# bnosac/image

Measured on NVIDIA H100. Metric: Mpixels/sec (Harris+Canny+HOG) at 4K frames, higher is better.
Workload: dtype f32 (Harris, FHOG) / f64 (Canny, Harris certification)

## Files before the change

image_b200/csrc/canny.cu:

```cuda
#include "common.cuh"
#include <cmath>
#include <vector>

namespace b2f {

constexpr int CANNY_MAXR = 64;
struct CannyTaps {
  double w[CANNY_MAXR + 1];
  int R;
};

constexpr int CB_TW = 32, CB_TH = 64, CB_NT = 256;

__device__ __forceinline__ int wrap_index(int p, int n) {
  while (p < 0) p += n;
  while (p >= n) p -= n;
  return p;
}

template <int RT>
__global__ void __launch_bounds__(CB_NT, 3)
canny_blur_kernel(const unsigned char *__restrict__ frames, float *__restrict__ out, int nx, int ny,
                  const __grid_constant__ CannyTaps tx, const __grid_constant__ CannyTaps ty) {
  extern __shared__ __align__(16) double smem_d[];
// ... 21 lines not shown
        for (int q = 0; q < MAXC; q++) b[k][q] = (lane + 32 * q < TILE_W) ? __ldg(row + cofs[q]) : (unsigned char)0;
      }
#pragma unroll
      for (int k = 0; k < RBATCH; k++) {
        const int r = r0 + (CB_NT / 32) * k;
        if (r < TILE_H) {
#pragma unroll
          for (int q = 0; q < MAXC; q++) if (lane + 32 * q < TILE_W) tile[r * TP + lane + 32 * q] = (double)b[k][q];
        }
      }
    }
    for (int r = warp; r < TILE_H; r += CB_NT / 32) {
      const unsigned char *row = src + (size_t)wrap_index(y0 - RY + r, ny) * nx;
      for (int c = lane + 32 * MAXC; c < TILE_W; c += 32) tile[r * TP + c] = (double)__ldg(row + wrap_index(x0 - RX + c, nx));
    }
  }
  __syncthreads();
  if (RT) {
    constexpr int RR = RT ? RT : 1;
    constexpr int NV = 4 + 2 * RR;
    for (int it = threadIdx.x; it < TILE_H * (CB_TW / 4); it += CB_NT) {
      const int r = it / (CB_TW / 4), g = it - r * (CB_TW / 4);
      const double *p = tile + r * TP + 4 * g;
      double v[NV];
#pragma unroll
      for (int q = 0; q < NV / 2; q++) { double2 t = *reinterpret_cast<const double2 *>(p + 2 * q); v[2 * q] = t.x; v[2 * q + 1] = t.y; }
      double o[4];
#pragma unroll
      for (int j = 0; j < 4; j++) {
        double acc = __dmul_rn(tx.w[0], v[j + RR]);
#pragma unroll
        for (int k = 1; k <= RR; k++) acc = __fma_rn(tx.w[k], __dadd_rn(v[j + RR - k], v[j + RR + k]), acc);
        o[j] = acc;
      }
      double *d = rowbuf + r * CB_TW + 4 * g;
      *reinterpret_cast<double2 *>(d) = make_double2(o[0], o[1]);
      *reinterpret_cast<double2 *>(d + 2) = make_double2(o[2], o[3]);
    }
  } else {
    for (int r = warp; r < TILE_H; r += CB_NT / 32) {
      const double *p = tile + r * TP + lane + RX;
      double acc = __dmul_rn(tx.w[0], p[0]);
      for (int k = 1; k <= RX; k++) acc = __fma_rn(tx.w[k], __dadd_rn(p[-k], p[k]), acc);
      rowbuf[r * CB_TW + lane] = acc;
    }
  }
  __syncthreads();
  {
    const int c = lane;
    const int gx = x0 + c;
    float *dst = out + (size_t)blockIdx.z * nx * ny;
    if (RT) {
      constexpr int RB = 8;
      constexpr int RR = RT ? RT : 1;
      for (int rg = warp; rg < CB_TH / RB; rg += CB_NT / 32) {
        double v[RB + 2 * RR];
#pragma unroll
        for (int q = 0; q < RB + 2 * RR; q++) v[q] = rowbuf[(rg * RB + q) * CB_TW + c];
#pragma unroll
        for (int j = 0; j < RB; j++) {
          double acc = __dmul_rn(ty.w[0], v[j + RR]);
#pragma unroll
          for (int k = 1; k <= RR; k++) acc = __fma_rn(ty.w[k], __dadd_rn(v[j + RR - k], v[j + RR + k]), acc);
          int gy = y0 + rg * RB + j;
          if (gx < nx && gy < ny) dst[(size_t)gy * nx + gx] = __double2float_rn(acc);
        }
      }
    } else {
      for (int r = warp; r < CB_TH; r += CB_NT / 32) {
        const double *p = rowbuf + (r + RY) * CB_TW + c;
        double acc = __dmul_rn(ty.w[0], p[0]);
        for (int k = 1; k <= RY; k++) acc = __fma_rn(ty.w[k], __dadd_rn(p[-k * CB_TW], p[k * CB_TW]), acc);
        int gy = y0 + r;
        if (gx < nx && gy < ny) dst[(size_t)gy * nx + gx] = __double2float_rn(acc);
      }
    }
  }
}

__device__ __forceinline__ double u32_to_double(unsigned s) {
  return __dadd_rn(__hiloint2double(0x43300000, (int)s), -4503599627370496.0);
}

template <int RR>
__global__ void __launch_bounds__(256)
canny_blur_rows_kernel(const unsigned char *__restrict__ frames, double *__restrict__ rowsum, int nx, int ny,
                       const __grid_constant__ CannyTaps tx) {
  const int y = blockIdx.y;
  const int x4 = (blockIdx.x * blockDim.x + threadIdx.x) * 4;
  if (x4 >= nx) return;
  const unsigned char *row = frames + ((size_t)blockIdx.z * ny + y) * nx;
  constexpr int LEAD = (RR + 3) & ~3;
  constexpr int NW = (LEAD + 4 + RR + 3) / 4;
  unsigned char b[NW * 4];
  const bool fast = (nx & 3) == 0 && NW * 4 <= nx && (reinterpret_cast<uintptr_t>(frames) & 3) == 0;
  if (fast) {
    const unsigned *w = reinterpret_cast<const unsigned *>(row);
    const int nw = nx >> 2, w0 = (x4 - LEAD) >> 2;
    unsigned v[NW];
#pragma unroll
    for (int q = 0; q < NW; q++) {
      int wi = w0 + q;
      wi += wi < 0 ? nw : 0;
      wi -= wi >= nw ? nw : 0;
      v[q] = __ldg(w + wi);
    }
#pragma unroll
    for (int q = 0; q < NW; q++) { b[4 * q] = v[q] & 0xff; b[4 * q + 1] = (v[q] >> 8) & 0xff; b[4 * q + 2] = (v[q] >> 16) & 0xff; b[4 * q + 3] = v[q] >> 24; }
  } else {
#pragma unroll
    for (int q = 0; q < NW * 4; q++) b[q] = __ldg(row + wrap_index(x4 - LEAD + q, nx));
  }
  double o[4];
#pragma unroll
  for (int j = 0; j < 4; j++) {
    const int c = LEAD + j;
    double acc = __dmul_rn(tx.w[0], u32_to_double(b[c]));
#pragma unroll
    for (int k = 1; k <= RR; k++) acc = __fma_rn(tx.w[k], u32_to_double((unsigned)b[c - k] + (unsigned)b[c + k]), acc);
    o[j] = acc;
  }
  double *d = rowsum + ((size_t)blockIdx.z * ny + y) * nx + x4;
  if (x4 + 3 < nx && (nx & 1) == 0) {
    *reinterpret_cast<double2 *>(d) = make_double2(o[0], o[1]);
    *reinterpret_cast<double2 *>(d + 2) = make_double2(o[2], o[3]);
  } else {
#pragma unroll
    for (int j = 0; j < 4; j++) if (x4 + j < nx) d[j] = o[j];
  }
}

constexpr int CC_TW = 32, CC_TH = 128;
template <int RR>
__global__ void __launch_bounds__(256)
canny_blur_cols_kernel(const double *__restrict__ rowsum, float *__restrict__ out, int nx, int ny,
                       const __grid_constant__ CannyTaps ty) {
  extern __shared__ __align__(16) double smem_d[];
  constexpr int TILE_H = CC_TH + 2 * RR;
  const int x0 = blockIdx.x * CC_TW, y0 = blockIdx.y * CC_TH;
  const double *src = rowsum + (size_t)blockIdx.z * nx * ny;
  const int lane = threadIdx.x & 31, warp = threadIdx.x >> 5;
  const int gx = x0 + lane;
  const int cx = min(gx, nx - 1);
  {
    constexpr int RBATCH = 10;
    for (int r0 = warp; r0 < TILE_H; r0 += 8 * RBATCH) {
      double v[RBATCH];
#pragma unroll
      for (int k = 0; k < RBATCH; k++) {
        const int r = min(r0 + 8 * k, TILE_H - 1);
        v[k] = __ldg(src + (size_t)wrap_index(y0 - RR + r, ny) * nx + cx);
      }
#pragma unroll
      for (int k = 0; k < RBATCH; k++) { const int r = r0 + 8 * k; if (r < TILE_H) smem_d[r * CC_TW + lane] = v[k]; }
    }
  }
  __syncthreads();
  float *dst = out + (size_t)blockIdx.z * nx * ny;
  constexpr int RB = 8;
  for (int rg = warp; rg < CC_TH / RB; rg += 8) {
    double v[RB + 2 * RR];
#pragma unroll
    for (int q = 0; q < RB + 2 * RR; q++) v[q] = smem_d[(rg * RB + q) * CC_TW + lane];
#pragma unroll
    for (int j = 0; j < RB; j++) {
      double acc = __dmul_rn(ty.w[0], v[j + RR]);
#pragma unroll
      for (int k = 1; k <= RR; k++) acc = __fma_rn(ty.w[k], __dadd_rn(v[j + RR - k], v[j + RR + k]), acc);
      const int gy = y0 + rg * RB + j;
      if (gx < nx && gy < ny) dst[(size_t)gy * nx + gx] = __double2float_rn(acc);
    }
  }
}

struct TapList { const int *coord; const double *weight; int n; int sym; };
__global__ void canny_blur_generic_rows(const unsigned char *__restrict__ frames, double *__restrict__ tmp, int nx, int ny,
                                        TapList t) {
  int x = blockIdx.x * blockDim.x + threadIdx.x, y = blockIdx.y;
  if (x >= nx) return;
  const unsigned char *src = frames + (size_t)blockIdx.z * nx * ny + (size_t)y * nx;
  double acc;
  if (t.sym) {
    const int R = t.n / 2;
    acc = __dmul_rn(t.weight[R], (double)src[x]);
    for (int k = 1; k <= R; k++)
      acc = __fma_rn(t.weight[R + k], __dadd_rn((double)src[wrap_index(x - k, nx)], (double)src[wrap_index(x + k, nx)]), acc);
  } else {
    acc = 0;
    for (int i = 0; i < t.n; i++) acc = __fma_rn(t.weight[i], (double)src[wrap_index(x - t.coord[i], nx)], acc);
  }
  tmp[(size_t)blockIdx.z * nx * ny + (size_t)y * nx + x] = acc;
}
__global__ void canny_blur_generic_cols(const double *__restrict__ tmp, float *__restrict__ out, int nx, int ny, TapList t) {
  int x = blockIdx.x * blockDim.x + threadIdx.x, y = blockIdx.y;
  if (x >= nx) return;
  const double *src = tmp + (size_t)blockIdx.z * nx * ny + x;
  double acc;
  if (t.sym) {
    const int R = t.n / 2;
    acc = __dmul_rn(t.weight[R], src[(size_t)y * nx]);
    for (int k = 1; k <= R; k++)
      acc = __fma_rn(t.weight[R + k], __dadd_rn(src[(size_t)wrap_index(y - k, ny) * nx], src[(size_t)wrap_index(y + k, ny) * nx]), acc);
  } else {
    acc = 0;
    for (int i = 0; i < t.n; i++) acc = __fma_rn(t.weight[i], src[(size_t)wrap_index(y - t.coord[i], ny) * nx], acc);
  }
  out[(size_t)blockIdx.z * nx * ny + (size_t)y * nx + x] = __double2float_rn(acc);
}

__device__ __forceinline__ double hypot_glibc(double x, double y) {
  x = fabs(x); y = fabs(y);
  double ax = x < y ? y : x, ay = x < y ? x : y;
  if (ax >= __dmul_rn(ay, 0x1p54)) return __dadd_rn(ax, ay);
  double h = __dsqrt_rn(__dadd_rn(__dmul_rn(ax, ax), __dmul_rn(ay, ay)));
  double t1, t2;
  if (h <= __dmul_rn(2.0, ay)) {
    double delta = __dsub_rn(h, ay);
    t1 = __dmul_rn(ax, __dsub_rn(__dmul_rn(2.0, delta), ax));
    t2 = __dmul_rn(__dsub_rn(delta, __dmul_rn(2.0, __dsub_rn(ax, ay))), delta);
  } else {
    double delta = __dsub_rn(h, ax);
    t1 = __dmul_rn(__dmul_rn(2.0, delta), __dsub_rn(ax, __dmul_rn(2.0, ay)));
    t2 = __dadd_rn(__dmul_rn(__dsub_rn(__dmul_rn(4.0, delta), ay), ay), __dmul_rn(delta, delta));
  }
  return __dsub_rn(h, __ddiv_rn(__dadd_rn(t1, t2), __dmul_rn(2.0, h)));
}

constexpr int CG_T = 32, CG_NT = 256;

constexpr int SG_DW = CG_T + 4;
constexpr int SG_DH = CG_T + 5;
constexpr int SG_GW = CG_T + 2;
constexpr int SG_GH = CG_T + 3;
constexpr int SG_K = 5;
__device__ __forceinline__ float rcp_approx(float x) { float r; asm("rcp.approx.ftz.f32 %0, %1;" : "=f"(r) : "f"(x)); return r; }
__device__ __forceinline__ float sqrt_approx(float x) { float r; asm("sqrt.approx.ftz.f32 %0, %1;" : "=f"(r) : "f"(x)); return r; }

__device__ __forceinline__ void exact_hv2(const float *d, int accGrad, double &h, double &v) {
#define DD(dx, dy) ((double)d[(dy) * SG_DW + (dx)])
  if (accGrad) {
    h = __dmul_rn(2.0, __dsub_rn(DD(1, 0), DD(-1, 0)));
    h = __dadd_rn(h, DD(1, 1)); h = __dsub_rn(h, DD(-1, 1)); h = __dadd_rn(h, DD(1, -1)); h = __dsub_rn(h, DD(-1, -1));
    v = __dmul_rn(2.0, __dsub_rn(DD(0, 1), DD(0, -1)));
    v = __dadd_rn(v, DD(1, 1)); v = __dsub_rn(v, DD(1, -1)); v = __dadd_rn(v, DD(-1, 1)); v = __dsub_rn(v, DD(-1, -1));
  } else {
    h = __dsub_rn(DD(1, 0), DD(-1, 0));
    v = __dsub_rn(DD(0, 1), DD(0, -1));
  }
#undef DD
}

template <bool ACC>
__global__ void __launch_bounds__(CG_NT)
canny_grad_nms_spec2_kernel(const float *__restrict__ data, unsigned *__restrict__ emask, unsigned *__restrict__ smask, int nx, int ny,
                            int low_thr, int high_thr, unsigned long long *__restrict__ fallback_count) {
  __shared__ __align__(16) float sd[SG_DH * SG_DW];
  __shared__ float fg[SG_GH * SG_GW];
  __shared__ float2 fhv[SG_GH * SG_GW];
  __shared__ float s_emax[CG_NT / 32];
  __shared__ __align__(4) unsigned char scls[CG_T * CG_T];
  __shared__ unsigned short squeue[CG_T * CG_T];
  __shared__ double sg2[28 * 9];
  __shared__ int qn;
  const int x0 = blockIdx.x * CG_T, y0 = blockIdx.y * CG_T;
  const float *src = data + (size_t)blockIdx.z * nx * ny;
  const int lane = threadIdx.x & 31, warp = threadIdx.x >> 5;
  if (threadIdx.x == 0) qn = 0;
  if (x0 >= 2 && y0 >= 2 && x0 + SG_DW - 2 <= nx && y0 + SG_DH - 2 <= ny && (nx & 1) == 0) {
    const float *org = src + (size_t)(y0 - 2) * nx + (x0 - 2);
    float2 v[3];
    int so[3];
#pragma unroll
    for (int k = 0; k < 3; k++) {
      const int u = threadIdx.x + k * CG_NT;
      const int row = u / (SG_DW / 2), cu = u - row * (SG_DW / 2);
      so[k] = row * SG_DW + 2 * cu;
      v[k] = u < SG_DH * (SG_DW / 2) ? __ldg(reinterpret_cast<const float2 *>(org + (size_t)row * nx + 2 * cu)) : make_float2(0.f, 0.f);
    }
#pragma unroll
    for (int k = 0; k < 3; k++)
      if (threadIdx.x + k * CG_NT < SG_DH * (SG_DW / 2)) *reinterpret_cast<float2 *>(sd + so[k]) = v[k];
  } else {
    const int c0 = min(max(x0 - 2 + lane, 0), nx - 1), c1 = min(max(x0 - 2 + lane + 32, 0), nx - 1);
    float a[5], b[5];
#pragma unroll
    for (int k = 0; k < 5; k++) {
      const int j = min(warp + 8 * k, SG_DH - 1);
      const float *row = src + (size_t)min(max(y0 - 2 + j, 0), ny - 1) * nx;
      a[k] = __ldg(row + c0);
      b[k] = lane < SG_DW - 32 ? __ldg(row + c1) : 0.f;
    }
#pragma unroll
    for (int k = 0; k < 5; k++) {
      const int j = warp + 8 * k;
      if (j < SG_DH) { sd[j * SG_DW + lane] = a[k]; if (lane < SG_DW - 32) sd[j * SG_DW + lane + 32] = b[k]; }
    }
  }
  __syncthreads();
  float emax = 0.f;
  if (threadIdx.x < 7 * SG_GW) {
    const int strip = threadIdx.x / SG_GW, c = threadIdx.x - strip * SG_GW;
    const float *d = sd + strip * SG_K * SG_DW + c;
    float l0 = d[0], m0 = d[1], q0 = d[2];
    float l1 = d[SG_DW], m1 = d[SG_DW + 1], q1 = d[SG_DW + 2];
    float dh0 = q0 - l0, dh1 = q1 - l1;
    int gi = strip * SG_K * SG_GW + c;
#pragma unroll
    for (int k = 0; k < SG_K; k++) {
      const float l2 = d[(k + 2) * SG_DW], m2 = d[(k + 2) * SG_DW + 1], q2 = d[(k + 2) * SG_DW + 2];
      const float dh2 = q2 - l2;
      float h, v, S;
      const float vy = m2 - m0;
      if (ACC) {
        const float vp = q2 - q0, vm = l2 - l0;
        h = fmaf(2.f, dh1, dh2 + dh0);
        v = fmaf(2.f, vy, vp + vm);
        S = fmaf(2.f, fabsf(dh1) + fabsf(vy), (fabsf(dh2) + fabsf(dh0)) + (fabsf(vp) + fabsf(vm)));
      } else {
        h = dh1; v = vy;
        S = fabsf(h) + fabsf(v);
      }
      const float g = sqrt_approx(fmaf(h, h, v * v));
      fg[gi + k * SG_GW] = g;
      fhv[gi + k * SG_GW] = make_float2(h, v);
      if (strip * SG_K + k < SG_GW) emax = fmaxf(emax, fmaf(6e-7f, S, 4e-7f * g));
      l0 = l1; m0 = m1; q0 = q1; dh0 = dh1;
      l1 = l2; m1 = m2; q1 = q2; dh1 = dh2;
    }
  }
  for (int o = 16; o; o >>= 1) emax = fmaxf(emax, __shfl_xor_sync(0xffffffffu, emax, o));
  if (lane == 0) s_emax[warp] = emax;
  __syncthreads();
  float E = s_emax[0];
#pragma unroll
  for (int w = 1; w < CG_NT / 32; w++) E = fmaxf(E, s_emax[w]);
  E = fmaxf(E, 1e-7f);
  const bool interior = x0 >= 1 && y0 >= 1 && x0 + CG_T + 1 <= nx && y0 + CG_T + 1 <= ny;
  const float lowf = (float)low_thr, highf = (float)high_thr;
  const float T0 = 2.f * E;
#pragma unroll
  for (int k = 0; k < CG_T * CG_T / CG_NT; k++) {
    const int t = threadIdx.x + k * CG_NT;
    const int ly = t >> 5, lx = t & 31;
    const int gx = x0 + lx, gy = y0 + ly;
    unsigned char c = 0;
    const int ci = (ly + 1) * SG_GW + lx + 1;
    const float now = fg[ci];
    if (gx < nx && gy < ny && now >= lowf - T0) {
      const float inv = rcp_approx(now);
      const float2 hv = fhv[ci];
      const float cs = hv.x * inv, sn = hv.y * inv;
      const float dcs = 8.f * fmaf(E, inv, 5e-7f);
      const int ngx = cs < 0.f, ngy = sn < 0.f;
      const float wbx = cs + (float)ngx, wax = 1.f - wbx, wby = sn + (float)ngy, way = 1.f - wby;
      float p11, p12, p21, p22, m11, m12, m21, m22;
      if (interior) {
        const float *gp = fg + ci - ngy * SG_GW - ngx;
        const float *gm = fg + ci + (ngy - 1) * SG_GW + (ngx - 1);
        p11 = gp[0]; p12 = gp[1]; p21 = gp[SG_GW]; p22 = gp[SG_GW + 1];
        m11 = gm[0]; m12 = gm[1]; m21 = gm[SG_GW]; m22 = gm[SG_GW + 1];
      } else {
        const int ox = x0 - 1, oy = y0 - 1;
        const int px1 = min(max(gx - ngx, 0), nx - 1) - ox, px2 = min(max(gx - ngx + 1, 0), nx - 1) - ox;
        const int py1 = min(max(gy - ngy, 0), ny - 1) - oy, py2 = min(max(gy - ngy + 1, 0), ny - 1) - oy;
        const int mx1 = min(max(gx + ngx - 1, 0), nx - 1) - ox, mx2 = min(max(gx + ngx, 0), nx - 1) - ox;
        const int my1 = min(max(gy + ngy - 1, 0), ny - 1) - oy, my2 = min(max(gy + ngy, 0), ny - 1) - oy;
        p11 = fg[py1 * SG_GW + px1]; p12 = fg[py1 * SG_GW + px2]; p21 = fg[py2 * SG_GW + px1]; p22 = fg[py2 * SG_GW + px2];
        m11 = fg[my1 * SG_GW + mx1]; m12 = fg[my1 * SG_GW + mx2]; m21 = fg[my2 * SG_GW + mx1]; m22 = fg[my2 * SG_GW + mx2];
      }
      const float nbp = way * fmaf(wax, p11, wbx * p12) + wby * fmaf(wax, p21, wbx * p22);
      const float nbm = wby * fmaf(wbx, m11, wax * m12) + way * fmaf(wbx, m21, wax * m22);
      const float spp = fmaxf(fmaxf(p11, p12), fmaxf(p21, p22)) - fminf(fminf(p11, p12), fminf(p21, p22));
      const float spm = fmaxf(fmaxf(m11, m12), fmaxf(m21, m22)) - fminf(fminf(m11, m12), fminf(m21, m22));
      const float tolp = fmaf(dcs, spp, 2.f * T0), tolm = fmaf(dcs, spm, 2.f * T0);
      const bool amb = now <= lowf + T0 || fminf(fabsf(cs), fabsf(sn)) <= dcs;
      const bool sup = now < fmaxf(nbp - tolp, nbm - tolm);
      const bool top = now > fmaxf(nbp + tolp, nbm + tolm);
      const bool hi2 = now >= highf + T0, hi1 = now < highf - T0;
      const bool undecided = amb || (!sup && (!top || (!hi2 && !hi1)));
      c = (!undecided && !sup) ? (hi2 ? 2 : 1) : 0;
      if (undecided) squeue[atomicAdd(&qn, 1)] = (unsigned short)t;
    }
    scls[t] = c;
  }
  __syncthreads();
  const int nq = qn;
  double *eg = sg2;
  for (int qb = 0; qb < nq; qb += 28) {
    const int nc = min(28, nq - qb);
    for (int i = threadIdx.x; i < nc * 9; i += CG_NT) {
      const int qi = i / 9, k = i - qi * 9;
      const int t = squeue[qb + qi], ly = t >> 5, lx = t & 31;
      const int px = min(max(x0 + lx + (k % 3) - 1, 0), nx - 1), py = min(max(y0 + ly + (k / 3) - 1, 0), ny - 1);
      double h, v;
      exact_hv2(sd + (py - (y0 - 2)) * SG_DW + (px - (x0 - 2)), ACC, h, v);
      eg[i] = hypot_glibc(h, v);
    }
    __syncthreads();
    for (int qi = threadIdx.x; qi < nc; qi += CG_NT) {
      const int t = squeue[qb + qi], ly = t >> 5, lx = t & 31;
      const int gx = x0 + lx, gy = y0 + ly;
      const double *g9 = eg + qi * 9;
      double h, v;
      exact_hv2(sd + (gy - (y0 - 2)) * SG_DW + (gx - (x0 - 2)), ACC, h, v);
      const double now = g9[4];
      unsigned char c;
      if (now <= (double)low_thr) c = 0;
      else {
        double sn, cs;
        if (h == 0.0 || v == 0.0) { const double th = atan2(v, h); sincos(th, &sn, &cs); }
        else { const double inv = __ddiv_rn(1.0, now); cs = __dmul_rn(h, inv); sn = __dmul_rn(v, inv); }
        double nb[2];
        for (int s2 = 0; s2 < 2; s2++) {
          const double dir = s2 ? 1.0 : -1.0;
          const double xt = __dmul_rn(dir, cs), yt = __dmul_rn(dir, sn);
          const double x1 = floor(xt), x2 = __dadd_rn(x1, 1.0), y1 = floor(yt), y2 = __dadd_rn(y1, 1.0);
          auto G = [&](double ox, double oy) -> double {
            const int ix = (int)ox, iy = (int)oy;
            if (ix > 1 || iy > 1) return 0.0;
            const int cxp = min(max(gx + ix, 0), nx - 1) - gx, cyp = min(max(gy + iy, 0), ny - 1) - gy;
            return g9[(cyp + 1) * 3 + (cxp + 1)];
          };
          const double wa = __dsub_rn(x2, xt), wb = __dsub_rn(xt, x1);
          const double g1 = __dadd_rn(__dmul_rn(wa, G(x1, y1)), __dmul_rn(wb, G(x2, y1)));
          const double g2 = __dadd_rn(__dmul_rn(wa, G(x1, y2)), __dmul_rn(wb, G(x2, y2)));
          nb[s2] = __dadd_rn(__dmul_rn(__dsub_rn(y2, yt), g1), __dmul_rn(__dsub_rn(yt, y1), g2));
        }
        if (now <= nb[0] || now <= nb[1]) c = 0;
        else c = now >= (double)high_thr ? 2 : 1;
      }
      scls[t] = c;
    }
    __syncthreads();
  }
  {
    const size_t t = ((size_t)blockIdx.z * gridDim.y + blockIdx.y) * gridDim.x + blockIdx.x;
#pragma unroll
    for (int k = 0; k < CG_T / (CG_NT / 32); k++) {
      const int ly = warp + (CG_NT / 32) * k;
      const unsigned char c = scls[ly * CG_T + lane];
      const unsigned e = __ballot_sync(0xffffffffu, c != 0), s = __ballot_sync(0xffffffffu, c == 2);
      if (lane == 0) { emask[CG_T * t + ly] = e; smask[CG_T * t + ly] = s; }
    }
  }
  if (fallback_count && threadIdx.x == 0 && nq) atomicAdd(fallback_count, (unsigned long long)nq);
}

__device__ __forceinline__ int uf_find(volatile int *L, int a) {
  int p = L[a];
  while (p != a) {
    int g = L[p];
    if (g != p) L[a] = g;
    a = p; p = g;
  }
  return a;
}
__device__ __forceinline__ int uf_find_ro(const volatile int *L, int a) {
  int p = L[a];
  while (p != a) { a = p; p = L[a]; }
  return a;
}
__device__ __forceinline__ void uf_union(int *L, int a, int b) {
  while (true) {
    a = uf_find(L, a); b = uf_find(L, b);
    if (a == b) return;
    if (a < b) { int t = a; a = b; b = t; }
    int old = atomicMin(&L[a], b);
    if (old == a) return;
    a = old;
  }
}

constexpr int HT = CG_T;
constexpr int HYST_MAX_RUNS = HT / 2;
constexpr int HYST_MAX_ROOTS = (HT / 2) * (HT / 2);

__device__ __forceinline__ int run_start(unsigned bits, int x) {
  return x - __clz(~(bits << (31 - x))) + 1;
}
__device__ __forceinline__ int run_ordinal(unsigned bits, int x) {
  return __popc(bits & ~(bits << 1) & (0xffffffffu >> (31 - x))) - 1;
}
__device__ __forceinline__ unsigned run_mask_from(unsigned bits, int s) {
  const unsigned t = ~(bits >> s);
  const int len = t ? __ffs(t) - 1 : 32;
  return (len >= 32 ? 0xffffffffu : ((1u << len) - 1u)) << s;
}

__global__ void __launch_bounds__(256)
hyst_local_kernel(const unsigned *__restrict__ E, const unsigned *__restrict__ S, unsigned char *__restrict__ runc,
                  int *__restrict__ ncomp, int *__restrict__ parent, unsigned char *__restrict__ strong, int n_tiles) {
  __shared__ int lab_all[8][HT * HYST_MAX_RUNS];
  __shared__ unsigned char num_all[8][HT * HYST_MAX_RUNS];
  __shared__ __align__(8) unsigned char cst_all[8][HYST_MAX_ROOTS];
  const int lane = threadIdx.x & 31, warp = threadIdx.x >> 5;
  const int tile = blockIdx.x * 8 + warp;
  if (tile >= n_tiles) return;
  int *lab = lab_all[warp];
  unsigned char *num = num_all[warp], *cst = cst_all[warp];
  const unsigned emask = E[(size_t)HT * tile + lane], smask = S[(size_t)HT * tile + lane];
  if (!__any_sync(0xffffffffu, emask != 0)) { if (lane == 0) ncomp[tile] = 0; return; }
  const int nr = __popc(emask & ~(emask << 1)), s0 = lane * HYST_MAX_RUNS;
  for (int j = 0; j < nr; j++) lab[s0 + j] = s0 + j;
  reinterpret_cast<uint2 *>(cst)[lane] = make_uint2(0, 0);
  const unsigned up = __shfl_up_sync(0xffffffffu, emask, 1);
  __syncwarp();
  if (lane > 0 && up) {
    int j = 0;
    for (unsigned rem = emask; rem; j++) {
      const unsigned low = rem & (0u - rem), x = rem + low, rm = rem & ~x;
      rem &= x;
      unsigned touch = up & (rm | (rm << 1) | (rm >> 1));
      while (touch) {
        const int us = run_start(up, __ffs(touch) - 1);
        const unsigned uhi = up >> us << us, ulow = 1u << us;
        touch &= ~(uhi & ~(uhi + ulow));
        uf_union(lab, s0 + j, s0 - HYST_MAX_RUNS + run_ordinal(up, us));
      }
    }
  }
  __syncwarp();
  unsigned isroot = 0;
  for (int j = 0; j < nr; j++) {
    const int rt = uf_find(lab, s0 + j);
    lab[s0 + j] = rt;
    isroot |= (unsigned)(rt == s0 + j) << j;
  }
  const int mine = __popc(isroot);
// ... 182 lines not shown
  for (int c = lo; c <= hi; c++) {
    double g = exp(-(double)c * c * inv_s * inv_s);
    if (g < 0x1p-64) continue;
    coord.push_back(c); weight.push_back(g / total);
  }
}
static bool symmetric_taps(const std::vector<int> &c, const std::vector<double> &w, CannyTaps &out) {
  int n = (int)c.size();
  if (n % 2 == 0) return false;
  int R = n / 2;
  if (R > CANNY_MAXR) return false;
  for (int k = 0; k <= R; k++) {
    if (c[R - k] != -k || c[R + k] != k || w[R - k] != w[R + k]) return false;
    out.w[k] = w[R + k];
  }
  out.R = R;
  return true;
}

static size_t hyst_scratch_bytes(size_t tiles) {
  return 2 * align256(tiles * HT * 4)  + align256(tiles * HT * HYST_MAX_RUNS)  +
         align256(tiles * 4)  + align256(tiles * HYST_MAX_ROOTS * 4)  + 2 * align256(tiles * HYST_MAX_ROOTS) ;
}
static size_t hyst_tile_count(int n_frames, int nx, int ny) { return (size_t)ceil_div(nx, HT) * ceil_div(ny, HT) * n_frames; }

size_t canny_scratch_bytes(int n_frames, int nx, int ny) {
  const size_t n = (size_t)n_frames * nx * ny;
  return align256(n * 4)  + hyst_scratch_bytes(hyst_tile_count(n_frames, nx, ny)) +
         align256(n * 8)  + (1 << 16) ;
}

static int canny_batch_geometry(const char *who, int n_frames, int nx, int ny, int *TX, int *TY, int *n_tiles) {
  if ((size_t)nx * ny * n_frames >= (size_t)1 << 31) {
    set_error("%s: batch of %d frames %dx%d exceeds 2^31 pixels; split the batch", who, n_frames, nx, ny);
    return B2F_EUNSUP;
  }
  const size_t tiles = hyst_tile_count(n_frames, nx, ny);
  if (tiles * HYST_MAX_ROOTS >= (size_t)1 << 31) {
    set_error("%s: batch of %d frames %dx%d has too many 32x32 tiles; split the batch", who, n_frames, nx, ny);
    return B2F_EUNSUP;
  }
  *TX = ceil_div(nx, HT); *TY = ceil_div(ny, HT); *n_tiles = (int)tiles;
  return B2F_OK;
}

static int canny_hysteresis(b2f_ctx *ctx, const unsigned *emask, const unsigned *smask, int n_frames, int nx, int ny, int TX,
                            int TY, int n_tiles, unsigned char *d_edges, int *d_nonzero, cudaStream_t st) {
  const size_t tiles = (size_t)n_tiles;
  unsigned char *runc = ctx->arena.get<unsigned char>(tiles * HT * HYST_MAX_RUNS);
  int *ncomp = ctx->arena.get<int>(tiles);
  int *parent = ctx->arena.get<int>(tiles * HYST_MAX_ROOTS);
  unsigned char *strong = ctx->arena.get<unsigned char>(tiles * HYST_MAX_ROOTS), *keep = ctx->arena.get<unsigned char>(tiles * HYST_MAX_ROOTS);
  B2F_ARENA_CHECK(ctx);
  B2F_CUDA(cudaMemsetAsync(d_nonzero, 0, sizeof(int) * n_frames, st));
  const unsigned hb = (unsigned)ceil_div(n_tiles, 8);
  hyst_local_kernel<<<hb, 256, 0, st>>>(emask, smask, runc, ncomp, parent, strong, n_tiles);
  B2F_LAUNCH_CHECK(ctx);
  hyst_seam_kernel<<<hb, 256, 0, st>>>(emask, runc, parent, TX, TY, n_tiles);
  B2F_LAUNCH_CHECK(ctx);
  hyst_mark_kernel<<<hb, 256, 0, st>>>(ncomp, parent, strong, n_tiles);
  B2F_LAUNCH_CHECK(ctx);
  hyst_resolve_kernel<<<hb, 256, 0, st>>>(ncomp, parent, strong, keep, n_tiles);
  B2F_LAUNCH_CHECK(ctx);
  const int vec = (nx % 16 == 0) && ((reinterpret_cast<uintptr_t>(d_edges) & 15) == 0);
  hyst_emit_kernel<<<hb, 256, 0, st>>>(emask, runc, keep, d_edges, d_nonzero, nx, ny, TX, TY, n_tiles, vec);
  B2F_LAUNCH_CHECK(ctx);
  return B2F_OK;
}

int canny_device(b2f_ctx *ctx, const unsigned char *d_frames, int n_frames, int nx, int ny, double s, double low_thr,
                 double high_thr, int acc_grad, unsigned char *d_edges, int *d_nonzero, cudaStream_t st) {
  const size_t n = (size_t)nx * ny * n_frames;
  int TX, TY, n_tiles;
  int rc = canny_batch_geometry("canny", n_frames, nx, ny, &TX, &TY, &n_tiles);
  if (rc != B2F_OK) return rc;
  if (!(s > 0)) { set_error("canny: s must be > 0"); return B2F_EINVAL; }
  const size_t tiles = (size_t)n_tiles;
  float *blur = ctx->arena.get<float>(n);
  unsigned *emask = ctx->arena.get<unsigned>(tiles * HT), *smask = ctx->arena.get<unsigned>(tiles * HT);
  std::vector<int> cx, cy; std::vector<double> wx, wy;
  make_taps(nx, s, cx, wx); make_taps(ny, s, cy, wy);
  CannyTaps tx, ty;
  const bool sym = symmetric_taps(cx, wx, tx) && symmetric_taps(cy, wy, ty);
  size_t smem = 0;
  if (sym) smem = sizeof(double) * ((size_t)(CB_TH + 2 * ty.R) * CB_TW + (size_t)(CB_TH + 2 * ty.R) * ((CB_TW + 2 * tx.R + 1) & ~1));
  if (sym && smem <= 200 * 1024) {
    B2F_ARENA_CHECK(ctx);
    dim3 grid(ceil_div(nx, CB_TW), ceil_div(ny, CB_TH), n_frames);
    static const bool tiled13 = getenv("B2F_CANNY_TILED_BLUR") != nullptr;
    if (tx.R == 13 && ty.R == 13 && !tiled13 && nx >= 64 && ny >= 64) {
      double *rowsum = ctx->arena.get<double>(n);
      B2F_ARENA_CHECK(ctx);
      canny_blur_rows_kernel<13><<<dim3(ceil_div(ceil_div(nx, 4), 256), ny, n_frames), 256, 0, st>>>(d_frames, rowsum, nx, ny, tx);
      B2F_LAUNCH_CHECK(ctx);
      const size_t csm = sizeof(double) * (size_t)(CC_TH + 26) * CC_TW;
      B2F_CUDA(cudaFuncSetAttribute(canny_blur_cols_kernel<13>, cudaFuncAttributeMaxDynamicSharedMemorySize, (int)csm));
      canny_blur_cols_kernel<13><<<dim3(ceil_div(nx, CC_TW), ceil_div(ny, CC_TH), n_frames), 256, csm, st>>>(rowsum, blur, nx, ny, ty);
    } else if (tx.R == 13 && ty.R == 13) {
      B2F_CUDA(cudaFuncSetAttribute(canny_blur_kernel<13>, cudaFuncAttributeMaxDynamicSharedMemorySize, (int)smem));
      canny_blur_kernel<13><<<grid, CB_NT, smem, st>>>(d_frames, blur, nx, ny, tx, ty);
    } else {
      B2F_CUDA(cudaFuncSetAttribute(canny_blur_kernel<0>, cudaFuncAttributeMaxDynamicSharedMemorySize, (int)smem));
      canny_blur_kernel<0><<<grid, CB_NT, smem, st>>>(d_frames, blur, nx, ny, tx, ty);
    }
    B2F_LAUNCH_CHECK(ctx);
  } else {
    double *tmp = ctx->arena.get<double>(n);
    int *dcx = ctx->arena.get<int>(cx.size() + cy.size());
    double *dwx = ctx->arena.get<double>(wx.size() + wy.size());
    B2F_ARENA_CHECK(ctx);
    B2F_CUDA(cudaMemcpyAsync(dcx, cx.data(), cx.size() * 4, cudaMemcpyHostToDevice, st));
    B2F_CUDA(cudaMemcpyAsync(dcx + cx.size(), cy.data(), cy.size() * 4, cudaMemcpyHostToDevice, st));
    B2F_CUDA(cudaMemcpyAsync(dwx, wx.data(), wx.size() * 8, cudaMemcpyHostToDevice, st));
    B2F_CUDA(cudaMemcpyAsync(dwx + wx.size(), wy.data(), wy.size() * 8, cudaMemcpyHostToDevice, st));
    B2F_CUDA(cudaStreamSynchronize(st));
    dim3 grid(ceil_div(nx, 128), ny, n_frames);
    canny_blur_generic_rows<<<grid, 128, 0, st>>>(d_frames, tmp, nx, ny, TapList{dcx, dwx, (int)cx.size(), sym ? 1 : 0});
    B2F_LAUNCH_CHECK(ctx);
    canny_blur_generic_cols<<<grid, 128, 0, st>>>(tmp, blur, nx, ny, TapList{dcx + cx.size(), dwx + wx.size(), (int)cy.size(), sym ? 1 : 0});
    B2F_LAUNCH_CHECK(ctx);
  }
  if (!ctx->canny_stats) {
    B2F_CUDA(cudaMalloc(&ctx->canny_stats, 8));
    B2F_CUDA(cudaMemsetAsync(ctx->canny_stats, 0, 8, st));
  }
  unsigned long long *fc = static_cast<unsigned long long *>(ctx->canny_stats);
  if (acc_grad)
    canny_grad_nms_spec2_kernel<true><<<dim3(TX, TY, n_frames), CG_NT, 0, st>>>(blur, emask, smask, nx, ny, (int)low_thr, (int)high_thr, fc);
  else
    canny_grad_nms_spec2_kernel<false><<<dim3(TX, TY, n_frames), CG_NT, 0, st>>>(blur, emask, smask, nx, ny, (int)low_thr, (int)high_thr, fc);
  B2F_LAUNCH_CHECK(ctx);
  return canny_hysteresis(ctx, emask, smask, n_frames, nx, ny, TX, TY, n_tiles, d_edges, d_nonzero, st);
}

}

using namespace b2f;

extern "C" {

int b2f_canny_stats(b2f_ctx *ctx, unsigned long long *tier2_pixels) {
  if (!ctx || !tier2_pixels) { set_error("b2f_canny_stats: NULL argument"); return B2F_EINVAL; }
  *tier2_pixels = 0;
  if (!ctx->canny_stats) return B2F_OK;
  B2F_CUDA(cudaSetDevice(ctx->device));
  B2F_CUDA(cudaMemcpyAsync(tier2_pixels, ctx->canny_stats, 8, cudaMemcpyDeviceToHost, ctx->stream));
  B2F_CUDA(cudaStreamSynchronize(ctx->stream));
  return B2F_OK;
}

int b2f_canny_dev(b2f_ctx *ctx, const uint8_t *d_frames, int n_frames, int nx, int ny, double s, double low_thr,
                  double high_thr, int acc_grad, uint8_t *d_edges, int *d_nonzero, void *stream) {
  if (!ctx || !d_frames || !d_edges || !d_nonzero || n_frames <= 0 || nx <= 0 || ny <= 0) { set_error("b2f_canny_dev: bad argument"); return B2F_EINVAL; }
  B2F_CUDA(cudaSetDevice(ctx->device));
  cudaStream_t st;
  int rc = stream_handoff(ctx, stream, &st);
  if (rc != B2F_OK) return rc;
  if ((rc = arena_reserve(ctx, canny_scratch_bytes(n_frames, nx, ny))) != B2F_OK) return rc;
  return canny_device(ctx, d_frames, n_frames, nx, ny, s, low_thr, high_thr, acc_grad, d_edges, d_nonzero, st);
}

int b2f_canny_hysteresis_dev(b2f_ctx *ctx, const uint8_t *d_cls, int n_frames, int nx, int ny, uint8_t *d_edges,
                             int *d_nonzero, void *stream) {
  if (!ctx || !d_cls || !d_edges || !d_nonzero || n_frames <= 0 || nx <= 0 || ny <= 0) { set_error("b2f_canny_hysteresis_dev: bad argument"); return B2F_EINVAL; }
  int TX, TY, n_tiles;
  int rc = canny_batch_geometry("b2f_canny_hysteresis_dev", n_frames, nx, ny, &TX, &TY, &n_tiles);
  if (rc != B2F_OK) return rc;
  B2F_CUDA(cudaSetDevice(ctx->device));
  cudaStream_t st;
  if ((rc = stream_handoff(ctx, stream, &st)) != B2F_OK) return rc;
  if ((rc = arena_reserve(ctx, hyst_scratch_bytes((size_t)n_tiles))) != B2F_OK) return rc;
  unsigned *emask = ctx->arena.get<unsigned>((size_t)n_tiles * HT), *smask = ctx->arena.get<unsigned>((size_t)n_tiles * HT);
  B2F_ARENA_CHECK(ctx);
  hyst_pack_kernel<<<dim3(TX, TY, n_frames), 256, 0, st>>>(d_cls, emask, smask, nx, ny);
  B2F_LAUNCH_CHECK(ctx);
  return canny_hysteresis(ctx, emask, smask, n_frames, nx, ny, TX, TY, n_tiles, d_edges, d_nonzero, st);
}

int b2f_canny_batch(b2f_ctx *ctx, const uint8_t *frames, int n_frames, int nx, int ny, double s, double low_thr,
                    double high_thr, int acc_grad, uint8_t *edges, int *nonzero) {
  if (!ctx || !frames || !edges || !nonzero || n_frames <= 0 || nx <= 0 || ny <= 0) { set_error("b2f_canny_batch: bad argument"); return B2F_EINVAL; }
  B2F_CUDA(cudaSetDevice(ctx->device));
  const size_t plane = (size_t)nx * ny, n = plane * n_frames;
  const int C = frames_per_chunk(ctx, plane, n_frames), NCH = ceil_div(n_frames, C);
  int rc = arena_reserve(ctx, canny_scratch_bytes(C, nx, ny) + 2 * align256(n) + align256(n_frames * 4));
  if (rc != B2F_OK) return rc;
  unsigned char *d_in = ctx->arena.get<unsigned char>(n), *d_out = ctx->arena.get<unsigned char>(n);
  int *d_nz = ctx->arena.get<int>(n_frames);
  B2F_ARENA_CHECK(ctx);
  const size_t mark = ctx->arena.off;
  cudaStream_t st = ctx->stream;
  if ((rc = pipe_prepare(ctx, 2 * NCH)) != B2F_OK) return rc;
  for (int c = 0; c < NCH; c++) {
    const int f0 = c * C, nf = std::min(C, n_frames - f0);
    cudaEvent_t e_in = ctx->events[2 * c], e_done = ctx->events[2 * c + 1];
    rc = B2F_OK;
    if (cudaMemcpyAsync(d_in + plane * f0, frames + plane * f0, plane * nf, cudaMemcpyHostToDevice, ctx->s_in) != cudaSuccess ||
        cudaEventRecord(e_in, ctx->s_in) != cudaSuccess || cudaStreamWaitEvent(st, e_in, 0) != cudaSuccess) rc = B2F_ECUDA;
    ctx->arena.off = mark;
    if (rc == B2F_OK) rc = canny_device(ctx, d_in + plane * f0, nf, nx, ny, s, low_thr, high_thr, acc_grad, d_out + plane * f0, d_nz + f0, st);
    if (rc == B2F_OK && (cudaEventRecord(e_done, st) != cudaSuccess || cudaStreamWaitEvent(ctx->s_out, e_done, 0) != cudaSuccess ||
                         cudaMemcpyAsync(edges + plane * f0, d_out + plane * f0, plane * nf, cudaMemcpyDeviceToHost, ctx->s_out) != cudaSuccess)) rc = B2F_ECUDA;
    if (rc != B2F_OK) {
      if (rc == B2F_ECUDA) set_error("b2f_canny_batch: CUDA error in chunk %d: %s", c, cudaGetErrorString(cudaGetLastError()));
      pipe_drain(ctx);
      return rc;
    }
  }
  if (cudaMemcpyAsync(nonzero, d_nz, sizeof(int) * n_frames, cudaMemcpyDeviceToHost, st) != cudaSuccess) {
    set_error("b2f_canny_batch: %s", cudaGetErrorString(cudaGetLastError()));
    pipe_drain(ctx);
    return B2F_ECUDA;
  }
// ... 10 lines not shown
```

Measured before the change: 18370.

## Fuse Canny Gaussian blur with gradient/NMS into one tiled kernel

For the radius-13 symmetric case, a single kernel now loads a u8 tile with halo, runs the row and column double-precision blur in shared memory, and then applies gradient/NMS to four vertically stacked tiles. The NMS scratch space is aliased onto the row-sum buffer. This removes the global round trips for the row sums and the float blur image, and drops two kernel launches. In exchange, the halo blur work is recomputed per tile column and shared-memory use is high, which may limit occupancy. The old separable row/column kernels are deleted.

New measurement: 20240 (median of 6 runs). 1.1x the previous value.

```diff
diff --git a/image_b200/csrc/canny.cu b/image_b200/csrc/canny.cu
--- a/image_b200/csrc/canny.cu
+++ b/image_b200/csrc/canny.cu
@@ -127,97 +127,6 @@
   return __dadd_rn(__hiloint2double(0x43300000, (int)s), -4503599627370496.0);
 }
 
-template <int RR>
-__global__ void __launch_bounds__(256)
-canny_blur_rows_kernel(const unsigned char *__restrict__ frames, double *__restrict__ rowsum, int nx, int ny,
-                       const __grid_constant__ CannyTaps tx) {
-  const int y = blockIdx.y;
-  const int x4 = (blockIdx.x * blockDim.x + threadIdx.x) * 4;
-  if (x4 >= nx) return;
-  const unsigned char *row = frames + ((size_t)blockIdx.z * ny + y) * nx;
-  constexpr int LEAD = (RR + 3) & ~3;
-  constexpr int NW = (LEAD + 4 + RR + 3) / 4;
-  unsigned char b[NW * 4];
-  const bool fast = (nx & 3) == 0 && NW * 4 <= nx && (reinterpret_cast<uintptr_t>(frames) & 3) == 0;
-  if (fast) {
-    const unsigned *w = reinterpret_cast<const unsigned *>(row);
-    const int nw = nx >> 2, w0 = (x4 - LEAD) >> 2;
-    unsigned v[NW];
-#pragma unroll
-    for (int q = 0; q < NW; q++) {
-      int wi = w0 + q;
-      wi += wi < 0 ? nw : 0;
-      wi -= wi >= nw ? nw : 0;
-      v[q] = __ldg(w + wi);
-    }
-#pragma unroll
-    for (int q = 0; q < NW; q++) { b[4 * q] = v[q] & 0xff; b[4 * q + 1] = (v[q] >> 8) & 0xff; b[4 * q + 2] = (v[q] >> 16) & 0xff; b[4 * q + 3] = v[q] >> 24; }
-  } else {
-#pragma unroll
-    for (int q = 0; q < NW * 4; q++) b[q] = __ldg(row + wrap_index(x4 - LEAD + q, nx));
-  }
-  double o[4];
-#pragma unroll
-  for (int j = 0; j < 4; j++) {
-    const int c = LEAD + j;
-    double acc = __dmul_rn(tx.w[0], u32_to_double(b[c]));
-#pragma unroll
-    for (int k = 1; k <= RR; k++) acc = __fma_rn(tx.w[k], u32_to_double((unsigned)b[c - k] + (unsigned)b[c + k]), acc);
-    o[j] = acc;
-  }
-  double *d = rowsum + ((size_t)blockIdx.z * ny + y) * nx + x4;
-  if (x4 + 3 < nx && (nx & 1) == 0) {
-    *reinterpret_cast<double2 *>(d) = make_double2(o[0], o[1]);
-    *reinterpret_cast<double2 *>(d + 2) = make_double2(o[2], o[3]);
-  } else {
-#pragma unroll
-    for (int j = 0; j < 4; j++) if (x4 + j < nx) d[j] = o[j];
-  }
-}
-
-constexpr int CC_TW = 32, CC_TH = 128;
-template <int RR>
-__global__ void __launch_bounds__(256)
-canny_blur_cols_kernel(const double *__restrict__ rowsum, float *__restrict__ out, int nx, int ny,
-                       const __grid_constant__ CannyTaps ty) {
-  extern __shared__ __align__(16) double smem_d[];
-  constexpr int TILE_H = CC_TH + 2 * RR;
-  const int x0 = blockIdx.x * CC_TW, y0 = blockIdx.y * CC_TH;
-  const double *src = rowsum + (size_t)blockIdx.z * nx * ny;
-  const int lane = threadIdx.x & 31, warp = threadIdx.x >> 5;
-  const int gx = x0 + lane;
-  const int cx = min(gx, nx - 1);
-  {
-    constexpr int RBATCH = 10;
-    for (int r0 = warp; r0 < TILE_H; r0 += 8 * RBATCH) {
-      double v[RBATCH];
-#pragma unroll
-      for (int k = 0; k < RBATCH; k++) {
-        const int r = min(r0 + 8 * k, TILE_H - 1);
-        v[k] = __ldg(src + (size_t)wrap_index(y0 - RR + r, ny) * nx + cx);
-      }
-#pragma unroll
-      for (int k = 0; k < RBATCH; k++) { const int r = r0 + 8 * k; if (r < TILE_H) smem_d[r * CC_TW + lane] = v[k]; }
-    }
-  }
-  __syncthreads();
-  float *dst = out + (size_t)blockIdx.z * nx * ny;
-  constexpr int RB = 8;
-  for (int rg = warp; rg < CC_TH / RB; rg += 8) {
-    double v[RB + 2 * RR];
-#pragma unroll
-    for (int q = 0; q < RB + 2 * RR; q++) v[q] = smem_d[(rg * RB + q) * CC_TW + lane];
-#pragma unroll
-    for (int j = 0; j < RB; j++) {
-      double acc = __dmul_rn(ty.w[0], v[j + RR]);
-#pragma unroll
-      for (int k = 1; k <= RR; k++) acc = __fma_rn(ty.w[k], __dadd_rn(v[j + RR - k], v[j + RR + k]), acc);
-      const int gy = y0 + rg * RB + j;
-      if (gx < nx && gy < ny) dst[(size_t)gy * nx + gx] = __double2float_rn(acc);
-    }
-  }
-}
-
 struct TapList { const int *coord; const double *weight; int n; int sym; };
 __global__ void canny_blur_generic_rows(const unsigned char *__restrict__ frames, double *__restrict__ tmp, int nx, int ny,
                                         TapList t) {
@@ -295,53 +204,28 @@
 #undef DD
 }
 
+struct NmsScratch {
+  double sg2[28 * 9];
+  float2 fhv[SG_GH * SG_GW];
+  float fg[SG_GH * SG_GW];
+  float s_emax[CG_NT / 32];
+  unsigned short squeue[CG_T * CG_T];
+  unsigned char scls[CG_T * CG_T];
+  int qn;
+};
+
 template <bool ACC>
-__global__ void __launch_bounds__(CG_NT)
-canny_grad_nms_spec2_kernel(const float *__restrict__ data, unsigned *__restrict__ emask, unsigned *__restrict__ smask, int nx, int ny,
-                            int low_thr, int high_thr, unsigned long long *__restrict__ fallback_count) {
-  __shared__ __align__(16) float sd[SG_DH * SG_DW];
-  __shared__ float fg[SG_GH * SG_GW];
-  __shared__ float2 fhv[SG_GH * SG_GW];
-  __shared__ float s_emax[CG_NT / 32];
-  __shared__ __align__(4) unsigned char scls[CG_T * CG_T];
-  __shared__ unsigned short squeue[CG_T * CG_T];
-  __shared__ double sg2[28 * 9];
-  __shared__ int qn;
-  const int x0 = blockIdx.x * CG_T, y0 = blockIdx.y * CG_T;
-  const float *src = data + (size_t)blockIdx.z * nx * ny;
+__device__ __forceinline__ void nms_tile(const float *sd, NmsScratch &ns, int x0, int y0, int nx, int ny, int low_thr,
+                                         int high_thr, unsigned *emask_t, unsigned *smask_t,
+                                         unsigned long long *fallback_count) {
+  float *fg = ns.fg, *s_emax = ns.s_emax;
+  float2 *fhv = ns.fhv;
+  unsigned char *scls = ns.scls;
+  unsigned short *squeue = ns.squeue;
+  double *sg2 = ns.sg2;
+  int &qn = ns.qn;
   const int lane = threadIdx.x & 31, warp = threadIdx.x >> 5;
   if (threadIdx.x == 0) qn = 0;
-  if (x0 >= 2 && y0 >= 2 && x0 + SG_DW - 2 <= nx && y0 + SG_DH - 2 <= ny && (nx & 1) == 0) {
-    const float *org = src + (size_t)(y0 - 2) * nx + (x0 - 2);
-    float2 v[3];
-    int so[3];
-#pragma unroll
-    for (int k = 0; k < 3; k++) {
-      const int u = threadIdx.x + k * CG_NT;
-      const int row = u / (SG_DW / 2), cu = u - row * (SG_DW / 2);
-      so[k] = row * SG_DW + 2 * cu;
-      v[k] = u < SG_DH * (SG_DW / 2) ? __ldg(reinterpret_cast<const float2 *>(org + (size_t)row * nx + 2 * cu)) : make_float2(0.f, 0.f);
-    }
-#pragma unroll
-    for (int k = 0; k < 3; k++)
-      if (threadIdx.x + k * CG_NT < SG_DH * (SG_DW / 2)) *reinterpret_cast<float2 *>(sd + so[k]) = v[k];
-  } else {
-    const int c0 = min(max(x0 - 2 + lane, 0), nx - 1), c1 = min(max(x0 - 2 + lane + 32, 0), nx - 1);
-    float a[5], b[5];
-#pragma unroll
-    for (int k = 0; k < 5; k++) {
-      const int j = min(warp + 8 * k, SG_DH - 1);
-      const float *row = src + (size_t)min(max(y0 - 2 + j, 0), ny - 1) * nx;
-      a[k] = __ldg(row + c0);
-      b[k] = lane < SG_DW - 32 ? __ldg(row + c1) : 0.f;
-    }
-#pragma unroll
-    for (int k = 0; k < 5; k++) {
-      const int j = warp + 8 * k;
-      if (j < SG_DH) { sd[j * SG_DW + lane] = a[k]; if (lane < SG_DW - 32) sd[j * SG_DW + lane + 32] = b[k]; }
-    }
-  }
-  __syncthreads();
   float emax = 0.f;
   if (threadIdx.x < 7 * SG_GW) {
     const int strip = threadIdx.x / SG_GW, c = threadIdx.x - strip * SG_GW;
@@ -478,17 +362,159 @@
     }
     __syncthreads();
   }
-  {
-    const size_t t = ((size_t)blockIdx.z * gridDim.y + blockIdx.y) * gridDim.x + blockIdx.x;
-#pragma unroll
-    for (int k = 0; k < CG_T / (CG_NT / 32); k++) {
-      const int ly = warp + (CG_NT / 32) * k;
-      const unsigned char c = scls[ly * CG_T + lane];
-      const unsigned e = __ballot_sync(0xffffffffu, c != 0), s = __ballot_sync(0xffffffffu, c == 2);
-      if (lane == 0) { emask[CG_T * t + ly] = e; smask[CG_T * t + ly] = s; }
-    }
+#pragma unroll
+  for (int k = 0; k < CG_T / (CG_NT / 32); k++) {
+    const int ly = warp + (CG_NT / 32) * k;
+    const unsigned char c = scls[ly * CG_T + lane];
+    const unsigned e = __ballot_sync(0xffffffffu, c != 0), s = __ballot_sync(0xffffffffu, c == 2);
+    if (lane == 0) { emask_t[ly] = e; smask_t[ly] = s; }
   }
   if (fallback_count && threadIdx.x == 0 && nq) atomicAdd(fallback_count, (unsigned long long)nq);
+}
+
+template <bool ACC>
+__global__ void __launch_bounds__(CG_NT)
+canny_grad_nms_spec2_kernel(const float *__restrict__ data, unsigned *__restrict__ emask, unsigned *__restrict__ smask, int nx, int ny,
+                            int low_thr, int high_thr, unsigned long long *__restrict__ fallback_count) {
+  __shared__ __align__(16) float sd[SG_DH * SG_DW];
+  __shared__ NmsScratch ns;
+  const int x0 = blockIdx.x * CG_T, y0 = blockIdx.y * CG_T;
+  const float *src = data + (size_t)blockIdx.z * nx * ny;
+  const int lane = threadIdx.x & 31, warp = threadIdx.x >> 5;
+  if (x0 >= 2 && y0 >= 2 && x0 + SG_DW - 2 <= nx && y0 + SG_DH - 2 <= ny && (nx & 1) == 0) {
+    const float *org = src + (size_t)(y0 - 2) * nx + (x0 - 2);
+    float2 v[3];
+    int so[3];
+#pragma unroll
+    for (int k = 0; k < 3; k++) {
+      const int u = threadIdx.x + k * CG_NT;
+      const int row = u / (SG_DW / 2), cu = u - row * (SG_DW / 2);
+      so[k] = row * SG_DW + 2 * cu;
+      v[k] = u < SG_DH * (SG_DW / 2) ? __ldg(reinterpret_cast<const float2 *>(org + (size_t)row * nx + 2 * cu)) : make_float2(0.f, 0.f);
+    }
+#pragma unroll
+    for (int k = 0; k < 3; k++)
+      if (threadIdx.x + k * CG_NT < SG_DH * (SG_DW / 2)) *reinterpret_cast<float2 *>(sd + so[k]) = v[k];
+  } else {
+    const int c0 = min(max(x0 - 2 + lane, 0), nx - 1), c1 = min(max(x0 - 2 + lane + 32, 0), nx - 1);
+    float a[5], b[5];
+#pragma unroll
+    for (int k = 0; k < 5; k++) {
+      const int j = min(warp + 8 * k, SG_DH - 1);
+      const float *row = src + (size_t)min(max(y0 - 2 + j, 0), ny - 1) * nx;
+      a[k] = __ldg(row + c0);
+      b[k] = lane < SG_DW - 32 ? __ldg(row + c1) : 0.f;
+    }
+#pragma unroll
+    for (int k = 0; k < 5; k++) {
+      const int j = warp + 8 * k;
+      if (j < SG_DH) { sd[j * SG_DW + lane] = a[k]; if (lane < SG_DW - 32) sd[j * SG_DW + lane + 32] = b[k]; }
+    }
+  }
+  __syncthreads();
+  const size_t t = ((size_t)blockIdx.z * gridDim.y + blockIdx.y) * gridDim.x + blockIdx.x;
+  nms_tile<ACC>(sd, ns, x0, y0, nx, ny, low_thr, high_thr, emask + CG_T * t, smask + CG_T * t, fallback_count);
+}
+
+constexpr int FB_NT = 4;
+constexpr int FB_DH = FB_NT * CG_T + 5;
+constexpr int FB_RH = FB_DH + 26;
+constexpr int FB_UW = 16;
+constexpr int FB_RB = 7;
+constexpr size_t FB_SMEM = sizeof(double) * FB_RH * SG_DW + sizeof(float) * FB_DH * SG_DW;
+static_assert(sizeof(NmsScratch) <= sizeof(double) * FB_RH * SG_DW, "NMS scratch must fit in the row sums");
+static_assert(4 * FB_RH * FB_UW <= sizeof(float) * FB_DH * SG_DW, "u8 tile must fit in the data tile");
+static_assert(FB_DH % FB_RB == 0, "column pass rows");
+
+template <bool ACC>
+__global__ void __launch_bounds__(CG_NT, 3)
+canny_blur_grad_nms_kernel(const unsigned char *__restrict__ frames, unsigned *__restrict__ emask, unsigned *__restrict__ smask,
+                           int nx, int ny, int TY, const __grid_constant__ CannyTaps tx, const __grid_constant__ CannyTaps ty,
+                           int low_thr, int high_thr, unsigned long long *__restrict__ fallback_count) {
+  constexpr int RR = 13;
+  extern __shared__ __align__(16) double smem_d[];
+  double *rs = smem_d;
+  NmsScratch &ns = *reinterpret_cast<NmsScratch *>(smem_d);
+  float *sd = reinterpret_cast<float *>(smem_d + FB_RH * SG_DW);
+  unsigned *u8w = reinterpret_cast<unsigned *>(sd);
+  const int x0 = blockIdx.x * CG_T, y0 = blockIdx.y * (FB_NT * CG_T);
+  const unsigned char *src = frames + (size_t)blockIdx.z * nx * ny;
+  if ((nx & 3) == 0 && (reinterpret_cast<uintptr_t>(frames) & 3) == 0) {
+    constexpr int PER = (FB_RH * FB_UW + CG_NT - 1) / CG_NT;
+    const unsigned *w = reinterpret_cast<const unsigned *>(src);
+    const int nw = nx >> 2, wq = (threadIdx.x & (FB_UW - 1)) + (x0 >> 2) - 4;
+    const int wi = wq < 0 ? wq + nw : wq >= nw ? wq - nw : wq;
+    unsigned v[PER];
+#pragma unroll
+    for (int k = 0; k < PER; k++) {
+      const int r = min((int)(threadIdx.x + k * CG_NT) / FB_UW, FB_RH - 1);
+      v[k] = __ldg(w + (size_t)wrap_index(y0 - 15 + r, ny) * nw + wi);
+    }
+#pragma unroll
+    for (int k = 0; k < PER; k++)
+      if (threadIdx.x + k * CG_NT < FB_RH * FB_UW) u8w[threadIdx.x + k * CG_NT] = v[k];
+  } else {
+    unsigned char *u8b = reinterpret_cast<unsigned char *>(u8w);
+    for (int i = threadIdx.x; i < FB_RH * FB_UW * 4; i += CG_NT) {
+      const int r = i / (FB_UW * 4), c = i - r * (FB_UW * 4);
+      u8b[i] = __ldg(src + (size_t)wrap_index(y0 - 15 + r, ny) * nx + wrap_index(x0 - 16 + c, nx));
+    }
+  }
+  __syncthreads();
+  for (int it = threadIdx.x; it < FB_RH * (SG_DW / 4); it += CG_NT) {
+    const int j = it / (SG_DW / 4), g = it - j * (SG_DW / 4);
+    const unsigned *p = u8w + j * FB_UW + g;
+    unsigned char b[32];
+#pragma unroll
+    for (int q = 0; q < 8; q++) {
+      const unsigned v = p[q];
+      b[4 * q] = v & 0xff; b[4 * q + 1] = (v >> 8) & 0xff; b[4 * q + 2] = (v >> 16) & 0xff; b[4 * q + 3] = v >> 24;
+    }
+    double o[4];
+#pragma unroll
+    for (int jj = 0; jj < 4; jj++) {
+      const int c = 14 + jj;
+      double acc = __dmul_rn(tx.w[0], u32_to_double(b[c]));
+#pragma unroll
+      for (int k = 1; k <= RR; k++) acc = __fma_rn(tx.w[k], u32_to_double((unsigned)b[c - k] + (unsigned)b[c + k]), acc);
+      o[jj] = acc;
+    }
+    double *d = rs + j * SG_DW + 4 * g;
+    *reinterpret_cast<double2 *>(d) = make_double2(o[0], o[1]);
+    *reinterpret_cast<double2 *>(d + 2) = make_double2(o[2], o[3]);
+  }
+  __syncthreads();
+  for (int it = threadIdx.x; it < SG_DW * (FB_DH / FB_RB); it += CG_NT) {
+    const int rg = it / SG_DW, c = it - rg * SG_DW;
+    double v[FB_RB + 2 * RR];
+#pragma unroll
+    for (int q = 0; q < FB_RB + 2 * RR; q++) v[q] = rs[(rg * FB_RB + q) * SG_DW + c];
+#pragma unroll
+    for (int j = 0; j < FB_RB; j++) {
+      double acc = __dmul_rn(ty.w[0], v[j + RR]);
+#pragma unroll
+      for (int k = 1; k <= RR; k++) acc = __fma_rn(ty.w[k], __dadd_rn(v[j + RR - k], v[j + RR + k]), acc);
+      sd[(rg * FB_RB + j) * SG_DW + c] = __double2float_rn(acc);
+    }
+  }
+  __syncthreads();
+  if (x0 < 2 || y0 < 2 || x0 + SG_DW - 2 > nx || y0 + FB_DH - 2 > ny) {
+    for (int i = threadIdx.x; i < FB_DH * SG_DW; i += CG_NT) {
+      const int r = i / SG_DW, c = i - r * SG_DW;
+      const int rr = min(max(y0 - 2 + r, 0), ny - 1) - (y0 - 2), cc = min(max(x0 - 2 + c, 0), nx - 1) - (x0 - 2);
+      if (rr != r || cc != c) sd[i] = sd[rr * SG_DW + cc];
+    }
+    __syncthreads();
+  }
+#pragma unroll 1
+  for (int k = 0; k < FB_NT; k++) {
+    const int tyk = blockIdx.y * FB_NT + k;
+    if (tyk >= TY) break;
+    if (k) __syncthreads();
+    const size_t t = ((size_t)blockIdx.z * TY + tyk) * gridDim.x + blockIdx.x;
+    nms_tile<ACC>(sd + k * CG_T * SG_DW, ns, x0, y0 + k * CG_T, nx, ny, low_thr, high_thr, emask + CG_T * t, smask + CG_T * t,
+                  fallback_count);
+  }
 }
 
 __device__ __forceinline__ int uf_find(volatile int *L, int a) {
@@ -837,21 +863,31 @@
   make_taps(nx, s, cx, wx); make_taps(ny, s, cy, wy);
   CannyTaps tx, ty;
   const bool sym = symmetric_taps(cx, wx, tx) && symmetric_taps(cy, wy, ty);
+  if (!ctx->canny_stats) {
+    B2F_CUDA(cudaMalloc(&ctx->canny_stats, 8));
+    B2F_CUDA(cudaMemsetAsync(ctx->canny_stats, 0, 8, st));
+  }
+  unsigned long long *fc = static_cast<unsigned long long *>(ctx->canny_stats);
+  const int lo = (int)low_thr, hi = (int)high_thr;
   size_t smem = 0;
   if (sym) smem = sizeof(double) * ((size_t)(CB_TH + 2 * ty.R) * CB_TW + (size_t)(CB_TH + 2 * ty.R) * ((CB_TW + 2 * tx.R + 1) & ~1));
+  if (sym && tx.R == 13 && ty.R == 13 && nx >= 64 && ny >= 64) {
+    B2F_ARENA_CHECK(ctx);
+    const dim3 grid(TX, ceil_div(TY, FB_NT), n_frames);
+    if (acc_grad) {
+      B2F_CUDA(cudaFuncSetAttribute(canny_blur_grad_nms_kernel<true>, cudaFuncAttributeMaxDynamicSharedMemorySize, (int)FB_SMEM));
+      canny_blur_grad_nms_kernel<true><<<grid, CG_NT, FB_SMEM, st>>>(d_frames, emask, smask, nx, ny, TY, tx, ty, lo, hi, fc);
+    } else {
+      B2F_CUDA(cudaFuncSetAttribute(canny_blur_grad_nms_kernel<false>, cudaFuncAttributeMaxDynamicSharedMemorySize, (int)FB_SMEM));
+      canny_blur_grad_nms_kernel<false><<<grid, CG_NT, FB_SMEM, st>>>(d_frames, emask, smask, nx, ny, TY, tx, ty, lo, hi, fc);
+    }
+    B2F_LAUNCH_CHECK(ctx);
+    return canny_hysteresis(ctx, emask, smask, n_frames, nx, ny, TX, TY, n_tiles, d_edges, d_nonzero, st);
+  }
   if (sym && smem <= 200 * 1024) {
     B2F_ARENA_CHECK(ctx);
     dim3 grid(ceil_div(nx, CB_TW), ceil_div(ny, CB_TH), n_frames);
-    static const bool tiled13 = getenv("B2F_CANNY_TILED_BLUR") != nullptr;
-    if (tx.R == 13 && ty.R == 13 && !tiled13 && nx >= 64 && ny >= 64) {
-      double *rowsum = ctx->arena.get<double>(n);
-      B2F_ARENA_CHECK(ctx);
-      canny_blur_rows_kernel<13><<<dim3(ceil_div(ceil_div(nx, 4), 256), ny, n_frames), 256, 0, st>>>(d_frames, rowsum, nx, ny, tx);
-      B2F_LAUNCH_CHECK(ctx);
-      const size_t csm = sizeof(double) * (size_t)(CC_TH + 26) * CC_TW;
-      B2F_CUDA(cudaFuncSetAttribute(canny_blur_cols_kernel<13>, cudaFuncAttributeMaxDynamicSharedMemorySize, (int)csm));
-      canny_blur_cols_kernel<13><<<dim3(ceil_div(nx, CC_TW), ceil_div(ny, CC_TH), n_frames), 256, csm, st>>>(rowsum, blur, nx, ny, ty);
-    } else if (tx.R == 13 && ty.R == 13) {
+    if (tx.R == 13 && ty.R == 13) {
       B2F_CUDA(cudaFuncSetAttribute(canny_blur_kernel<13>, cudaFuncAttributeMaxDynamicSharedMemorySize, (int)smem));
       canny_blur_kernel<13><<<grid, CB_NT, smem, st>>>(d_frames, blur, nx, ny, tx, ty);
     } else {
@@ -875,15 +911,10 @@
     canny_blur_generic_cols<<<grid, 128, 0, st>>>(tmp, blur, nx, ny, TapList{dcx + cx.size(), dwx + wx.size(), (int)cy.size(), sym ? 1 : 0});
     B2F_LAUNCH_CHECK(ctx);
   }
-  if (!ctx->canny_stats) {
-    B2F_CUDA(cudaMalloc(&ctx->canny_stats, 8));
-    B2F_CUDA(cudaMemsetAsync(ctx->canny_stats, 0, 8, st));
-  }
-  unsigned long long *fc = static_cast<unsigned long long *>(ctx->canny_stats);
   if (acc_grad)
-    canny_grad_nms_spec2_kernel<true><<<dim3(TX, TY, n_frames), CG_NT, 0, st>>>(blur, emask, smask, nx, ny, (int)low_thr, (int)high_thr, fc);
+    canny_grad_nms_spec2_kernel<true><<<dim3(TX, TY, n_frames), CG_NT, 0, st>>>(blur, emask, smask, nx, ny, lo, hi, fc);
   else
-    canny_grad_nms_spec2_kernel<false><<<dim3(TX, TY, n_frames), CG_NT, 0, st>>>(blur, emask, smask, nx, ny, (int)low_thr, (int)high_thr, fc);
+    canny_grad_nms_spec2_kernel<false><<<dim3(TX, TY, n_frames), CG_NT, 0, st>>>(blur, emask, smask, nx, ny, lo, hi, fc);
   B2F_LAUNCH_CHECK(ctx);
   return canny_hysteresis(ctx, emask, smask, n_frames, nx, ny, TX, TY, n_tiles, d_edges, d_nonzero, st);
 }
```
